# j-dong/rust-raytrace

Measured on AMD Instinct MI355X. Metric: Mrays/sec at 4096x4096, 1000 spheres, depth 8; fraction of HBM roofline, higher is better.
Workload: dtype f64

## Files before the change

include/raytrace_amd.h:

```cpp
#ifndef RAYTRACE_AMD_H
#define RAYTRACE_AMD_H

#include <stddef.h>
#include <stdint.h>

#ifdef __cplusplus
extern "C" {
#endif

#define RT_ABI_VERSION 8

enum rt_status {
    RT_OK = 0,
    RT_E_INVALID = -1,
    RT_E_NODEVICE = -2,
    RT_E_HIP = -3,
    RT_E_NOMEM = -4,
    RT_E_UNSUPPORTED = -5,
    RT_E_PARSE = -6,
    RT_E_NOSCENE = -7,
    RT_E_IO = -8
};

enum rt_shape_kind { RT_SHAPE_SPHERE = 0, RT_SHAPE_PLANE = 1 };
enum rt_material_kind {
    RT_MAT_PHONG = 0, RT_MAT_INDIRECT_PHONG = 1, RT_MAT_FRESNEL = 2, RT_MAT_TRANSPARENT = 3
};
enum rt_light_kind { RT_LIGHT_POINT = 0, RT_LIGHT_DIRECTIONAL = 1, RT_LIGHT_AREA = 2 };
enum rt_camera_kind { RT_CAMERA_SIMPLE = 0, RT_CAMERA_DOF = 1 };
enum rt_background_kind { RT_BG_SOLID = 0, RT_BG_SKYBOX = 1 };

typedef struct { double r, g, b; } rt_color;

// ... 124 lines not shown
void rt_render_opts_default(rt_render_opts* o, uint32_t width, uint32_t height);

int rt_render(rt_ctx* ctx, const rt_render_opts* opts, float* out_rgb, uint8_t* out_bgr, rt_stats* stats);
int rt_render_device(rt_ctx* ctx, const rt_render_opts* opts, void* d_rgb, void* d_bgr, void* stream);
int rt_ctx_reserve(rt_ctx* ctx, const rt_render_opts* opts, int host, void* stream);
int rt_ctx_stats(rt_ctx* ctx, rt_stats* stats);
typedef struct rt_accum rt_accum;

int rt_accum_create(rt_ctx* ctx, const rt_render_opts* opts, rt_accum** out);
void rt_accum_destroy(rt_accum* acc);
int rt_accum_samples(const rt_accum* acc, uint32_t* samples);
int rt_accum_reset(rt_accum* acc);
int rt_render_accumulate(rt_ctx* ctx, rt_accum* acc, uint32_t n_samples, int32_t algo, uint32_t flags, void* stream);
int rt_accum_resolve(rt_ctx* ctx, rt_accum* acc, uint32_t bgr_pitch, void* d_rgb, void* d_bgr, void* stream);
int rt_accum_resolve_host(rt_ctx* ctx, rt_accum* acc, uint32_t bgr_pitch, float* out_rgb, uint8_t* out_bgr);
int rt_accum_download(rt_ctx* ctx, rt_accum* acc, double* sums, size_t cap_doubles, uint32_t* samples);
int rt_accum_upload(rt_ctx* ctx, rt_accum* acc, const double* sums, size_t n_doubles, uint32_t samples);
int rt_checkpoint_write(const char* path, const rt_render_opts* opts, uint64_t scene_hash, uint32_t samples, const double* sums, size_t n_doubles);
int rt_checkpoint_read(const char* path, rt_render_opts* opts, uint64_t* scene_hash, uint32_t* samples, double* sums, size_t cap_doubles);
int rt_div_a2_check(rt_ctx* ctx, const double* x, const double* a, uint32_t n, double* fast, double* slow);
int rt_sqrt_check(rt_ctx* ctx, const double* x, uint32_t n, double* fast, double* slow);
int rt_cull_check(rt_ctx* ctx, uint32_t n, const double* rays, const float* boxes, const double* t, const int32_t* codes,
                  double reach, int32_t* out_i, float* out_f);
double rt_cull_reach(double extent);
int rt_ctx_generation_counts(rt_ctx* ctx, uint32_t* queue, uint32_t* shaded, int n);
enum rt_kernel_family {
    RT_KF_NEAREST = 0,
    RT_KF_OCCLUSION = 1,
    RT_KF_SHADE = 2,
    RT_KF_FOLD = 3,
    RT_KF_TALLY = 4,
    RT_KF_CAMERA = 5,
    RT_KF_COMPOSE = 6,
    RT_KF_TAIL = 7,
    RT_KF_COUNT = 8
};
int rt_ctx_kernel_times(rt_ctx* ctx, double* ms, uint32_t* launches, int n);

int rt_ctx_set_tuning(rt_ctx* ctx, const char* key, int64_t value);
int rt_ctx_get_tuning(const rt_ctx* ctx, const char* key, int64_t* value);
const char* rt_tuning_key(int index);

#ifdef __cplusplus
}
#endif
#endif
// ... 1 lines not shown
```

rust-raytrace_amd/csrc/launch_api.hpp:

```cpp
#pragma once
#include <hip/hip_runtime.h>

#include <cstdint>
#include <vector>

#include "device_layout.hpp"

namespace rtamd {

enum KernelFamily : int8_t {
    kKfNearest = 0, kKfOcclusion = 1, kKfShade = 2, kKfFold = 3, kKfTally = 4, kKfCamera = 5, kKfCompose = 6, kKfTail = 7, kKfCount = 8
};

struct LaunchInterval {
    int start, end;
    KernelFamily fam;
};

struct LaunchMarks {
    std::vector<hipEvent_t>* pool = nullptr;
    int* used = nullptr;
    std::vector<LaunchInterval>* out = nullptr;
    int prev = -1;
    static constexpr int kMaxEvents = 1 << 16;
// ... 44 lines not shown
    hipEvent_t sp_cam = nullptr, sp_ready = nullptr;
    uint32_t *sp_bits = nullptr, *sp_cnt = nullptr, *sp_off = nullptr;
    uint8_t* sp_bgr = nullptr;
    float* sp_rgb = nullptr;
};
hipError_t launch_wavefront(const DevScene& sc, const FrameParams& fp, const WfBufs& b, int src, int src_occ,
                            bool count, const WfStreams& ws, hipEvent_t mark, int mark_gen);
hipError_t upload_srgb_table(const double* avg255);
hipError_t launch_tally(const FrameParams& fp, const WfBufs& b, int n_lights, int generations, hipStream_t s);
constexpr int kDjFlags = 4, kDjWords = 8;
hipError_t launch_signal(uint64_t* flag, uint64_t n, hipStream_t s);
hipError_t launch_join(uint64_t* flags, uint32_t mask, uint64_t n, uint64_t* err, hipStream_t s);
constexpr uint32_t kSegPx = 16;
hipError_t launch_chain_segs(const FrameParams& fp, const WfBufs& b, uint32_t* segbits, uint32_t* rowcnt, uint32_t* rowoff,
                             hipStream_t s);
hipError_t launch_chain_pack(const FrameParams& fp, const uint32_t* segbits, const uint32_t* rowoff, uint8_t* pk_bgr,
                             float* pk_rgb, hipStream_t s);
hipError_t launch_warmup(uint32_t workgroups, hipStream_t s);
hipError_t launch_path_warmup(hipStream_t s);
hipError_t launch_div_a2_probe(const double* x, const double* a, uint32_t n, double* fast, double* slow, hipStream_t s);
hipError_t launch_sqrt_probe(const double* x, uint32_t n, double* fast, double* slow, hipStream_t s);
hipError_t launch_cull_probe(uint32_t n, const double* rays, const float* boxes, const double* t, const int32_t* codes,
                             float reach, int32_t* out_i, float* out_f, hipStream_t s);

size_t path_lds_bytes(const DevScene& sc, bool staged);
int path_waves_per_simd();
hipError_t launch_path(const DevScene& sc, const FrameParams& fp, const PathStack& st, bool staged, hipStream_t stream,
                       bool accumulate = false);
hipError_t launch_accum_resolve(const FrameParams& fp, uint32_t workgroups, hipStream_t s);

}
```

rust-raytrace_amd/csrc/probes.hip:

```cpp
#include <hip/hip_runtime.h>

#include <algorithm>
#include <cstdint>

#include "device_layout.hpp"
#include "launch_api.hpp"
#include "trace_common.hpp"
#include "wf_launch.hpp"

namespace rtamd {

__global__ __launch_bounds__(256) void div_a2_probe(const double* x, const double* a, uint32_t n, double* fast,
                                                    double* slow) {
    for (uint32_t i = blockIdx.x * 256u + threadIdx.x; i < n; i += gridDim.x * 256u) {
        const SphK k = sphere_k(a[i]);
        fast[i] = div_a2(x[i], k);
        slow[i] = x[i] / (2.0 * a[i]);
    }
}

__global__ __launch_bounds__(256) void sqrt_probe(const double* x, uint32_t n, double* fast, double* slow) {
    for (uint32_t i = blockIdx.x * 256u + threadIdx.x; i < n; i += gridDim.x * 256u) {
        fast[i] = sqrt_win(x[i]);
        slow[i] = sqrt(x[i]);
    }
}

__global__ __launch_bounds__(256) void cull_probe(uint32_t n, const double* rays, const float* boxes, const double* t,
                                                  const int32_t* codes, float reach, int32_t* out_i, float* out_f) {
    for (uint32_t i = blockIdx.x * 256u + threadIdx.x; i < n; i += gridDim.x * 256u) {
        const double* q = rays + 6ull * i;
        Ray r;
        r.ox = q[0]; r.oy = q[1]; r.oz = q[2]; r.dx = q[3]; r.dy = q[4]; r.dz = q[5];
        const float* B = boxes + 6ull * i;
        const float lo[3] = {B[0], B[1], B[2]}, hi[3] = {B[3], B[4], B[5]};
        const RayBox rb = make_raybox(r, reach);
        const float tl = t_limit(rb, t[i]);
        float tn, tn_nf;
        const bool hit = box_hit(lo, hi, rb, tl, tn);
        const bool lx = near_is_lo(rb.ix), ly = near_is_lo(rb.iy), lz = near_is_lo(rb.iz);
        const bool hit_nf = box_hit_nf(lx ? lo[0] : hi[0], ly ? lo[1] : hi[1], lz ? lo[2] : hi[2], lx ? hi[0] : lo[0],
                                       ly ? hi[1] : lo[1], lz ? hi[2] : lo[2], rb, tl, tn_nf);
        const uint32_t e16 = stk_entry_c<16>(codes[i], tn), e18 = stk_entry_c<18>(codes[i], tn);
        int32_t* oi = out_i + 5ull * i;
        float* of = out_f + 5ull * i;
        oi[0] = rb.te; oi[1] = hit ? 1 : 0; oi[2] = hit_nf ? 1 : 0; oi[3] = stk_node_c<16>(e16); oi[4] = stk_node_c<18>(e18);
        of[0] = tl; of[1] = tn; of[2] = tn_nf; of[3] = stk_t_c<16>(e16); of[4] = stk_t_c<18>(e18);
    }
}

hipError_t launch_cull_probe(uint32_t n, const double* rays, const float* boxes, const double* t, const int32_t* codes,
                             float reach, int32_t* out_i, float* out_f, hipStream_t s) {
    const uint32_t blocks = std::max(1u, std::min(4096u, (n + 255u) / 256u));
    hipLaunchKernelGGL(cull_probe, dim3(blocks), dim3(256), 0, s, n, rays, boxes, t, codes, reach, out_i, out_f);
    return hipGetLastError();
}

hipError_t launch_sqrt_probe(const double* x, uint32_t n, double* fast, double* slow, hipStream_t s) {
    const uint32_t blocks = std::max(1u, std::min(4096u, (n + 255u) / 256u));
    hipLaunchKernelGGL(sqrt_probe, dim3(blocks), dim3(256), 0, s, x, n, fast, slow);
    return hipGetLastError();
}

hipError_t launch_div_a2_probe(const double* x, const double* a, uint32_t n, double* fast, double* slow, hipStream_t s) {
    const uint32_t blocks = std::max(1u, std::min(4096u, (n + 255u) / 256u));
    hipLaunchKernelGGL(div_a2_probe, dim3(blocks), dim3(256), 0, s, x, a, n, fast, slow);
    return hipGetLastError();
}

RT_UNIT_WARM(probes)

}
```

rust-raytrace_amd/csrc/rt_device.cpp:

```cpp
#include <cstring>
#include <new>
#include <string>

#include "rt_ctx.hpp"

using namespace rtamd;

extern "C" {

int rt_device_count(int* n) {
    if (!n) return RT_E_INVALID;
    *n = 0;
    int k = 0;
    hipError_t e = hipGetDeviceCount(&k);
    if (e != hipSuccess) { *n = 0; return RT_OK; }
    *n = k;
    return RT_OK;
}

int rt_ctx_create(int device, rt_ctx** out) {
    if (!out) return RT_E_INVALID;
    *out = nullptr;
    int n = 0;
    if (hipGetDeviceCount(&n) != hipSuccess || device < 0 || device >= n)
// ... 95 lines not shown
        const size_t o_t = 48 * N, o_box = o_t + 8 * N, o_code = o_box + 24 * N, o_oi = o_code + 4 * N, o_of = o_oi + 20 * N;
        uint8_t* d = nullptr;
        HIP_TRY(c, hipMalloc(&d, o_of + 20 * N));
        auto body = [&]() -> int {
            HIP_TRY(c, hipMemcpyAsync(d, rays, 48 * N, hipMemcpyHostToDevice, c->stream));
            HIP_TRY(c, hipMemcpyAsync(d + o_t, t, 8 * N, hipMemcpyHostToDevice, c->stream));
            HIP_TRY(c, hipMemcpyAsync(d + o_box, boxes, 24 * N, hipMemcpyHostToDevice, c->stream));
            HIP_TRY(c, hipMemcpyAsync(d + o_code, codes, 4 * N, hipMemcpyHostToDevice, c->stream));
            HIP_TRY(c, launch_cull_probe(n, reinterpret_cast<const double*>(d), reinterpret_cast<const float*>(d + o_box),
                                         reinterpret_cast<const double*>(d + o_t), reinterpret_cast<const int32_t*>(d + o_code),
                                         static_cast<float>(reach), reinterpret_cast<int32_t*>(d + o_oi), reinterpret_cast<float*>(d + o_of),
                                         c->stream));
            HIP_TRY(c, hipMemcpyAsync(out_i, d + o_oi, 20 * N, hipMemcpyDeviceToHost, c->stream));
            HIP_TRY(c, hipMemcpyAsync(out_f, d + o_of, 20 * N, hipMemcpyDeviceToHost, c->stream));
            HIP_TRY(c, hipStreamSynchronize(c->stream));
            return RT_OK;
        };
        const int rc = body();
        (void)hipFree(d);
        return rc;
    });
}

int rt_sqrt_check(rt_ctx* c, const double* x, uint32_t n, double* fast, double* slow) {
    if (!c || (n && (!x || !fast || !slow))) return RT_E_INVALID;
    if (n == 0) return RT_OK;
    return guarded(c, [&] {
        HIP_TRY(c, hipSetDevice(c->device));
        const size_t bytes = static_cast<size_t>(n) * sizeof(double);
        double* d = nullptr;
        HIP_TRY(c, hipMalloc(&d, 3 * bytes));
        auto body = [&]() -> int {
            HIP_TRY(c, hipMemcpyAsync(d, x, bytes, hipMemcpyHostToDevice, c->stream));
            HIP_TRY(c, launch_sqrt_probe(d, n, d + n, d + 2 * static_cast<size_t>(n), c->stream));
            HIP_TRY(c, hipMemcpyAsync(fast, d + n, bytes, hipMemcpyDeviceToHost, c->stream));
            HIP_TRY(c, hipMemcpyAsync(slow, d + 2 * static_cast<size_t>(n), bytes, hipMemcpyDeviceToHost, c->stream));
            HIP_TRY(c, hipStreamSynchronize(c->stream));
            return RT_OK;
        };
        const int rc = body();
        (void)hipFree(d);
        return rc;
    });
}

int rt_ctx_set_tuning(rt_ctx* c, const char* key, int64_t value) {
// ... 27 lines not shown
```

rust-raytrace_amd/csrc/trace_common.hpp:

```cpp
#pragma once

#include <hip/hip_runtime.h>

#include <cstdint>
#include <type_traits>

#include "device_layout.hpp"

namespace rtamd {

#ifdef RT_UNIT
#define RT_CAT_(a, b) a##b
#define RT_CAT(a, b) RT_CAT_(a, b)
#define c_srgb_avg RT_CAT(c_srgb_avg_, RT_UNIT)
__constant__ double c_srgb_avg[255];
#else
extern __constant__ double c_srgb_avg[255];
#endif

constexpr double kMinSignificance = 1.0 / 256.0 / 2.0;
constexpr double kEps = 0.00001;
constexpr double kFrac1Pi = 0.318309886183790671537767526745028724;

struct Ray {
// ... 1062 lines not shown
    const double px = ((static_cast<double>(x) + jx) - fp.hw) * fp.scale;
    const double py = ((static_cast<double>(y) + jy) - fp.hh) * fp.scale;
    const double* M = sc.cam_m;
    const double dx = M[0] * px + M[1] * py + M[2] * 1.0;
    const double dy = M[3] * px + M[4] * py + M[5] * 1.0;
    const double dz = M[6] * px + M[7] * py + M[8] * 1.0;
#if RT_DIVK
    const DivK l = div_k(sqrt_win(dx * dx + dy * dy + dz * dz));
    return Ray{sc.cam_pos[0], sc.cam_pos[1], sc.cam_pos[2], div_by(dx, l), div_by(dy, l), div_by(dz, l)};
#else
    const double l = sqrt(dx * dx + dy * dy + dz * dz);
    return Ray{sc.cam_pos[0], sc.cam_pos[1], sc.cam_pos[2], dx / l, dy / l, dz / l};
#endif
}

__device__ __forceinline__ Ray reflect_ray(const Ray& r, double ptx, double pty, double ptz, double nx, double ny,
                                           double nz) {
    const double dn = r.dx * nx + r.dy * ny + r.dz * nz;
    const double k2 = 2.0 * dn;
    const double rdx = r.dx - nx * k2, rdy = r.dy - ny * k2, rdz = r.dz - nz * k2;
    return Ray{ptx + rdx * kEps, pty + rdy * kEps, ptz + rdz * kEps, rdx, rdy, rdz};
}

__device__ __forceinline__ Col average_samples(Col c, uint32_t spp) {
    c = Col{(0.0 + c.r) / 1.0, (0.0 + c.g) / 1.0, (0.0 + c.b) / 1.0};
    Col res{0.0, 0.0, 0.0};
    for (uint32_t k = 0; k < spp; ++k) res = Col{res.r + c.r, res.g + c.g, res.b + c.b};
    const double aa = static_cast<double>(spp);
    return Col{res.r / aa, res.g / aa, res.b / aa};
}

__device__ __forceinline__ void write_pixel(const FrameParams& fp, uint32_t lx, uint32_t out_row, Col res,
                                            const double* srgb = c_srgb_avg) {
    const size_t p = static_cast<size_t>(out_row) * fp.tile_w + lx;
    if (fp.out_rgb) {
        fp.out_rgb[3 * p + 0] = static_cast<float>(res.r);
        fp.out_rgb[3 * p + 1] = static_cast<float>(res.g);
        fp.out_rgb[3 * p + 2] = static_cast<float>(res.b);
    }
    if (fp.out_bgr) {
        uint8_t* q = fp.out_bgr + static_cast<size_t>(out_row) * fp.bgr_pitch + 3u * lx;
        q[0] = to_srgb(res.b, srgb);
        q[1] = to_srgb(res.g, srgb);
        q[2] = to_srgb(res.r, srgb);
        if (lx == fp.tile_w - 1)
            for (uint32_t k = 3u * fp.tile_w; k < fp.pad_end; ++k)
                fp.out_bgr[static_cast<size_t>(out_row) * fp.bgr_pitch + k] = 0;
    }
// ... 60 lines not shown
```

rust-raytrace_amd/csrc/wf_device.hpp:

```cpp
#pragma once
#include <hip/hip_runtime.h>

#include <cstdint>

#include "device_layout.hpp"
#include "trace_common.hpp"

namespace rtamd {
namespace {


__device__ __forceinline__ uint32_t lds_append(uint32_t* counter, bool want) {
    const unsigned long long mask = __ballot(want);
    if (mask == 0) return 0xFFFFFFFFu;
    const int lane = threadIdx.x & 63;
    const int leader = __ffsll(static_cast<long long>(mask)) - 1;
    uint32_t base = 0;
    if (lane == leader) base = atomicAdd(counter, static_cast<uint32_t>(__popcll(mask)));
    base = __shfl(base, leader, 64);
    const uint32_t below = static_cast<uint32_t>(__popcll(mask & ((1ull << lane) - 1ull)));
    return want ? base + below : 0xFFFFFFFFu;
}

__device__ __forceinline__ bool deal_major(const WfBufs& b, uint32_t n) { return b.wg_major && n >= b.spread_below; }
// ... 33 lines not shown
    __syncthreads();
    if (t == 0) {
        uint32_t acc = 0;
        for (int w = 0; w < kT / 64; ++w) { const uint32_t x = s_wave[w]; s_wave[w] = acc; acc += x; }
    }
    __syncthreads();
    uint32_t run = s_wave[wave] + inc - sum;
    for (uint32_t e = 0; e < per; ++e) {
        const uint32_t i = t * per + e;
        if (i < G) s_scan[i] = run;
        run += v[e];
    }
    if (t == kT - 1) s_scan[G] = run;
    __syncthreads();
}

__device__ __forceinline__ size_t region_entry(const uint32_t* s_scan, uint32_t G, uint32_t R, uint32_t i) {
    uint32_t lo = 0, hi = G - 1;
    while (lo < hi) {
        const uint32_t mid = (lo + hi + 1) >> 1;
        if (s_scan[mid] <= i) lo = mid; else hi = mid - 1;
    }
    return static_cast<size_t>(lo) * R + (i - s_scan[lo]);
}

__device__ __forceinline__ bool slot_pixel(const WfBufs& b, const FrameParams& fp, uint32_t j, uint32_t& lx, uint32_t& ly) {
    const uint32_t tile = j >> 6, w = j & 63u;
    lx = (tile % b.tiles_x) * 8u + (w & 7u);
    ly = (tile / b.tiles_x) * 8u + (w >> 3);
    return lx < fp.tile_w && ly < fp.rows;
}

#ifndef RT_NT
#define RT_NT 1
#endif
template <class T>
__device__ __forceinline__ T ldn(const T* p) {
#if RT_NT
    return __builtin_nontemporal_load(p);
#else
    return *p;
#endif
}
template <class T, class U>
__device__ __forceinline__ void stn(T* p, U v) {
#if RT_NT
// ... 356 lines not shown
```

rust-raytrace_amd/csrc/wf_fold.hip:

```cpp
#define RT_UNIT wf_fold
#include <hip/hip_runtime.h>

#include <cstdint>

#include "wf_chain.hpp"
#include "wf_launch.hpp"

namespace rtamd {

namespace {

template <bool kFresnel, bool kAa = false, bool kPack = false>
__global__ __launch_bounds__(RT_FOLD_THREADS, RT_FOLD_WAVES) void wf_fold(DevScene sc, FrameParams fp, WfBufs b, uint32_t lo,
                                                                          uint32_t hi) {
    constexpr int kT = RT_FOLD_THREADS;
    __shared__ double s_srgb[255];
    __shared__ uint32_t s_scan[kMaxRegions + 1];
    __shared__ uint32_t s_wave[kT / 64];
    for (int i = threadIdx.x; i < 255; i += kT) s_srgb[i] = c_srgb_avg[i];
    region_scan<kT>(b.rs(), b.G, s_scan, s_wave);
    const uint32_t n = s_scan[b.G];
    const uint32_t W = gridDim.x * (kT / 64), lane = threadIdx.x & 63u;
    struct Head {
        uint32_t c, nlev, p;
        Col term;
    };
    auto head = [&](uint64_t j) {
        Head hd{0u, kNlevRunning, 0u, Col{0.0, 0.0, 0.0}};
        if (j < n) {
            hd.c = static_cast<uint32_t>(region_entry(s_scan, b.G, b.R, static_cast<uint32_t>(j)));
            hd.nlev = b.nlev()[hd.c];
            hd.p = b.compose ? 0u : b.cpix()[hd.c];
            hd.term = Col{ldn_if<kNtFold>(&b.term(0)[hd.c]), ldn_if<kNtFold>(&b.term(1)[hd.c]),
                          ldn_if<kNtFold>(&b.term(2)[hd.c])};
        }
        return hd;
    };
    uint32_t rc = blockIdx.x * (kT / 64) + (threadIdx.x >> 6);
    Head cur = head(static_cast<uint64_t>(rc) * 64u + lane);
    for (; static_cast<uint64_t>(rc) * 64u < n; rc += W) {
        const Head nxt = head(static_cast<uint64_t>(rc + W) * 64u + lane);
        if (cur.nlev >= lo && cur.nlev <= hi) {
            const Col folded = fold_levels<kFresnel, kPack>(sc, b, cur.c, static_cast<int>(cur.nlev), cur.term);
            const Col res = kAa ? aa_sample(folded) : average_samples(folded, fp.spp);
            emit_chain<kAa>(fp, b, cur.c, cur.p, res, s_srgb);
        }
        cur = nxt;
    }
}

__global__ __launch_bounds__(RT_FOLD_THREADS) void wf_sky_term(DevScene sc, WfBufs b) {
    constexpr int kT = RT_FOLD_THREADS;
    __shared__ uint32_t s_scan[kMaxRegions + 1];
    __shared__ uint32_t s_wave[kT / 64];
    region_scan<kT>(b.rs(), b.G, s_scan, s_wave);
    const uint32_t n = s_scan[b.G];
    for (uint64_t j = static_cast<uint64_t>(blockIdx.x) * kT + threadIdx.x; j < n; j += static_cast<uint64_t>(gridDim.x) * kT) {
        const uint32_t c = static_cast<uint32_t>(region_entry(s_scan, b.G, b.R, static_cast<uint32_t>(j)));
        const uint32_t nl = b.nlev()[c];
        if (nl == kNlevRunning || !(nl & kNlevSky)) continue;
        const Col col = background(sc, Ray{0.0, 0.0, 0.0, b.term(0)[c], b.term(1)[c], b.term(2)[c]});
        b.term(0)[c] = col.r; b.term(1)[c] = col.g; b.term(2)[c] = col.b;
        b.nlev()[c] = static_cast<uint8_t>(nl & ~kNlevSky);
    }
}

}

hipError_t launch_fold(const DevScene& sc, const FrameParams& fp, const WfBufs& b, hipStream_t s, LaunchMarks* m,
                       uint32_t lo, uint32_t hi, bool packed) {
    hipError_t e;
    const dim3 grid(b.G * (kWfThreads / RT_FOLD_THREADS)), block(RT_FOLD_THREADS);
    if (sc.skybox) {
        if (m && (e = m->begin(s)) != hipSuccess) return e;
        hipLaunchKernelGGL(wf_sky_term, grid, block, 0, s, sc, b);
        if (m && (e = m->mark(s, kKfCompose)) != hipSuccess) return e;
    }
    if (m && (e = m->begin(s)) != hipSuccess) return e;
    (void)dispatch_bools(
        [&](auto kFresnel, auto kAa, auto kPack) {
            hipLaunchKernelGGL((wf_fold<kFresnel(), kAa(), kPack()>), grid, block, 0, s, sc, fp, b, lo, hi);
// ... 11 lines not shown
```

rust-raytrace_amd/csrc/wf_nearest.hpp:

```cpp
#pragma once
#include "wf_device.hpp"
#include "wf_launch.hpp"

namespace rtamd {

#ifndef RT_STAMP
#define RT_STAMP 0
#endif
#if RT_STAMP
static __device__ unsigned long long g_stamp[kMaxGenerations][12];
static __device__ unsigned long long g_stamp2[kMaxGenerations][4];
#define RT_STAMP_AT(v)                                                            \
    do {                                                                          \
        asm volatile("s_waitcnt vmcnt(0) lgkmcnt(0)" ::: "memory");              \
        v = __builtin_amdgcn_s_memtime();                                         \
    } while (0)
#define RT_UNIT_STAMPS(unit)                                                                                          \
    hipError_t unit_stamps_##unit(unsigned long long (*a)[12], unsigned long long (*b)[4], bool reset) {              \
        hipError_t e;                                                                                                 \
        if ((e = hipMemcpyFromSymbol(a, HIP_SYMBOL(g_stamp), sizeof g_stamp)) != hipSuccess) return e;                \
        if ((e = hipMemcpyFromSymbol(b, HIP_SYMBOL(g_stamp2), sizeof g_stamp2)) != hipSuccess) return e;              \
        if (!reset) return hipSuccess;                                                                                \
        static unsigned long long za[kMaxGenerations][12], zb[kMaxGenerations][4];                                    \
        if ((e = hipMemcpyToSymbol(HIP_SYMBOL(g_stamp), za, sizeof za)) != hipSuccess) return e;                      \
// ... 39 lines not shown
                double nx, ny, nz;
                hit_normal(sc, sph, h.prim, ptx, pty, ptz, nx, ny, nz);
                const double nd = nx * r.dx + ny * r.dy + nz * r.dz;
                const Shading sh = shading_flags<kFresnel>(m, sig, nd);
                if (!sh.diffuse && !sh.specular) {
                    ends = true;
                    end_obj = h.obj;
                } else {
                    shade = true;
                    if (sh.specular) {
                        if (nd > 0.0) { nx = -nx; ny = -ny; nz = -nz; }
                        rr = reflect_ray(r, ptx, pty, ptz, nx, ny, nz);
                        nsig = (sh.f * sig) * m.ks_sig;
                        refl = true;
                    }
                }
            }
        }
    }
    if (ends) {
        if constexpr (kCam) {
            if (b.compose) stn(&b.pmap()[p], kPixAmbient | static_cast<uint32_t>(end_obj));
            else if constexpr (kAa) aa_add(fp, p, aa_sample(end_colour(sc, end_obj)));
            else write_pixel(fp, p % fp.tile_w, fp.row0 + p / fp.tile_w, average_samples(end_colour(sc, end_obj), fp.spp));
        } else {
            set_terminal(b, p, end_colour(sc, end_obj), k);
        }
    }
    if constexpr (kCam) {
        if (b.mark && live) stn(&b.cmark()[p], static_cast<uint8_t>(shade ? 1 : 0));
        if constexpr (kSky) {
            if (!b.compose && live) stn(&b.csky()[p], static_cast<uint8_t>(h.obj == INT32_MAX ? 1 : 0));
        }
    }
    const uint32_t slot = lds_append(&counts[0], shade);
    const uint32_t chain = kCam ? static_cast<uint32_t>(obase) + slot : p;
    if (kCam && shade && b.compose) stn(&b.pmap()[p], chain);
    if (shade) {
        const size_t at = rbase + slot;
        stn(&b.rf(0)[at], ptx); stn(&b.rf(1)[at], pty); stn(&b.rf(2)[at], ptz);
        stn(&b.rf(3)[at], r.dx); stn(&b.rf(4)[at], r.dy); stn(&b.rf(5)[at], r.dz);
        stn(&b.rf(6)[at], sig);
        stn(&b.ru(0)[at], static_cast<uint32_t>(h.obj));
        stn(&b.ru(1)[at], static_cast<uint32_t>(h.prim));
        stn(&b.ru(2)[at], chain);
        stn(&b.ru(3)[at], 0u);
        if constexpr (kCam) {
// ... 134 lines not shown
```

rust-raytrace_amd/csrc/wf_shade.hip:

```cpp
#include <hip/hip_runtime.h>

#include <cstdint>

#include "wf_chain.hpp"
#include "wf_launch.hpp"

namespace rtamd {

namespace {

template <int kSrc, bool kCount>
__global__ __launch_bounds__(kWfThreads, Src<kSrc>::waves) void wf_occlusion(DevScene sc, FrameParams fp, WfBufs b, int k) {
    extern __shared__ __attribute__((aligned(16))) unsigned char lds[];
    const QueueLds ql = queue_lds(lds + staged_bytes<kSrc>(sc), b.G);
    region_scan(b.rs() + k * b.G, b.G, ql.scan, ql.wave);
    const uint32_t L = static_cast<uint32_t>(sc.n_lights);
    const uint32_t nrec = ql.scan[b.G], n = nrec * L;
    if (!wg_has_work(b, n)) return;
    const BvhView v = stage_lds<kSrc>(sc, lds);
    __syncthreads();
    Work w;
    const size_t rk = static_cast<size_t>(k) * b.qcap;
    const uint32_t W = b.G * (kWfThreads / 64), lane = threadIdx.x & 63u;
    auto item_at = [&](uint32_t qi, uint32_t& l) {
        l = qi / nrec;
        return rk + region_entry(ql.scan, b.G, b.R, qi - l * nrec);
    };
    uint32_t rc = wave_slot(b, n), lc = 0;
    size_t atc = 0;
    double pc[3] = {0.0, 0.0, 0.0};
    int32_t hc = -1;
    if (static_cast<uint64_t>(rc) * 64u + lane < n) {
        atc = item_at(rc * 64u + lane, lc);
        pc[0] = ldn_if<3>(&b.rf(0)[atc]); pc[1] = ldn_if<3>(&b.rf(1)[atc]); pc[2] = ldn_if<3>(&b.rf(2)[atc]);
        hc = static_cast<int32_t>(b.ru(1)[atc]);
    }
    for (; static_cast<uint64_t>(rc) * 64u < n; rc += W) {
        const uint64_t qn = static_cast<uint64_t>(rc + W) * 64u + lane;
        uint32_t ln = 0;
        size_t atn = 0;
        double pn[3] = {0.0, 0.0, 0.0};
        int32_t hn = -1;
        if (qn < n) {
            atn = item_at(static_cast<uint32_t>(qn), ln);
            pn[0] = ldn_if<3>(&b.rf(0)[atn]); pn[1] = ldn_if<3>(&b.rf(1)[atn]); pn[2] = ldn_if<3>(&b.rf(2)[atn]);
            hn = static_cast<int32_t>(b.ru(1)[atn]);
        }
        const uint32_t qi = rc * 64u + lane;
        const uint32_t l = lc;
        const size_t at = atc;
        const double ptx = pc[0], pty = pc[1], ptz = pc[2];
        const int32_t hint = hc;
        lc = ln; atc = atn; pc[0] = pn[0]; pc[1] = pn[1]; pc[2] = pn[2]; hc = hn;
        if (qi >= n) continue;
        double lx, ly, lz, r2;
        const bool has_range = light_dir(sc.lights[l], ptx, pty, ptz, lx, ly, lz, r2);
        const Ray sray{ptx + lx * kEps, pty + ly * kEps, ptz + lz * kEps, lx, ly, lz};
        bool occluded;
        if constexpr (Src<kSrc>::grid)
            occluded = occluded_lgrid<kCount>(sc, v, sc.lgrid[l], sray, r2, ptx, pty, ptz, hint, &w);
        else
            occluded = has_range && sc.lgrid && sc.lgrid[l].R > 0
                           ? occluded_lgrid<kCount>(sc, v, sc.lgrid[l], sray, r2, ptx, pty, ptz, hint, &w)
                           : occluded_any<kSrc, kCount>(sc, v, sray, has_range, r2, hint, &w);
        if (occluded) atomicOr(&b.ru(3)[at], 1u << l);
    }
    flush_work<kCount>(b, 4, w);
}

template <bool kFresnel, bool kPack = false>
__global__ __launch_bounds__(kWfThreads, RT_SHADE_WAVES) void wf_shade(DevScene sc, FrameParams fp, WfBufs b, int k) {
    __shared__ uint32_t s_scan[kMaxRegions + 1];
    __shared__ uint32_t s_wave[kWfThreads / 64];
    region_scan(b.rs() + k * b.G, b.G, s_scan, s_wave);
    const uint32_t n = s_scan[b.G];
    const size_t rk = static_cast<size_t>(k) * b.qcap;
    const uint32_t W = gridDim.x * (kWfThreads / 64), lane = threadIdx.x & 63u;
    const bool lit = sc.n_lights > 0;
    uint32_t rc = wave_slot(b, n);
    ShadeIn cur{};
    bool have = false;
    if (static_cast<uint64_t>(rc) * 64u + lane < n) {
        cur = shade_load(b, rk + region_entry(s_scan, b.G, b.R, rc * 64u + lane), lit);
        have = true;
    }
    for (; static_cast<uint64_t>(rc) * 64u < n; rc += W) {
        const uint64_t jn = static_cast<uint64_t>(rc + W) * 64u + lane;
        ShadeIn nxt{};
        const bool have_n = jn < n;
        if (have_n) nxt = shade_load(b, rk + region_entry(s_scan, b.G, b.R, static_cast<uint32_t>(jn)), lit);
        if (have) shade_compute<kFresnel, true, kPack>(sc, b, k, cur);
        cur = nxt;
        have = have_n;
    }
}

template <int kSrc>
hipError_t launch_occlusion_src(const DevScene& sc, const FrameParams& fp, const WfBufs& b, int k, bool count, hipStream_t s) {
    const size_t lds = staged_bytes<kSrc>(sc) + queue_lds_bytes(b.G);
    return dispatch_bools(
        [&](auto kCount) {
            hipLaunchKernelGGL((wf_occlusion<kSrc, kCount()>), dim3(b.G), dim3(kWfThreads), lds, s, sc, fp, b, k);
            return hipSuccess;
        },
        count);
}

}

hipError_t launch_shading(const DevScene& sc, const FrameParams& fp, const WfBufs& b, int k, int src_occ, int grid_occ,
                          bool count, bool packed, hipStream_t sb, LaunchMarks* mb) {
    hipError_t e;
    if (sc.n_lights > 0) {
// ... 28 lines not shown
```

rust-raytrace_amd/libraytrace/__init__.py:

```python
import ctypes as C
import os

import numpy as np

_HERE = os.path.dirname(os.path.abspath(__file__))
PKG_DIR = os.path.dirname(_HERE)
LIB_PATH = os.environ.get("RT_LIBRTAMD") or os.path.join(PKG_DIR, "librtamd.so")
HEADER_PATH = os.path.join(os.path.dirname(PKG_DIR), "include", "raytrace_amd.h")

RT_ABI_VERSION = 8
RT_OK = 0
RT_E_INVALID, RT_E_NODEVICE, RT_E_HIP, RT_E_NOMEM = -1, -2, -3, -4
RT_E_UNSUPPORTED, RT_E_PARSE, RT_E_NOSCENE, RT_E_IO = -5, -6, -7, -8
RT_SHAPE_SPHERE, RT_SHAPE_PLANE = 0, 1
RT_MAT_PHONG, RT_MAT_INDIRECT_PHONG, RT_MAT_FRESNEL, RT_MAT_TRANSPARENT = 0, 1, 2, 3
RT_LIGHT_POINT, RT_LIGHT_DIRECTIONAL, RT_LIGHT_AREA = 0, 1, 2
RT_CAMERA_SIMPLE, RT_CAMERA_DOF = 0, 1
RT_BG_SOLID, RT_BG_SKYBOX = 0, 1
RT_OUT_RGB_F32, RT_OUT_BGR_U8, RT_COUNT_WORK, RT_TIME_KERNELS, RT_OUT_FRAME_ROWS = 1, 2, 4, 8, 16
KERNEL_FAMILIES = ("nearest", "occlusion", "shade", "fold", "tally", "camera", "compose", "tail")
RT_ALGO_AUTO, RT_ALGO_BRUTE_LDS, RT_ALGO_BRUTE_GLOBAL, RT_ALGO_WAVEFRONT, RT_ALGO_WAVEFRONT_BRUTE = 0, 1, 2, 3, 4
RT_ALGO_PATH = 5
RT_ALGO_WAVEFRONT_AA = 6
RT_JITTER_CENTER, RT_JITTER_RANDOM = 0, 1
RT_MAX_DEPTH_LIMIT = 30


class RtError(RuntimeError):
    def __init__(self, code, msg):
        super().__init__(f"rt error {code}: {msg}")
        self.code = code


# ... 79 lines not shown
        "rt_render_accumulate": (C.c_int, [C.c_void_p, C.c_void_p, C.c_uint32, C.c_int32, C.c_uint32, C.c_void_p]),
        "rt_accum_resolve": (C.c_int, [C.c_void_p, C.c_void_p, C.c_uint32, C.c_void_p, C.c_void_p, C.c_void_p]),
        "rt_accum_resolve_host": (C.c_int, [C.c_void_p, C.c_void_p, C.c_uint32, P(C.c_float), P(C.c_uint8)]),
        "rt_accum_download": (C.c_int, [C.c_void_p, C.c_void_p, P(C.c_double), C.c_size_t, P(C.c_uint32)]),
        "rt_accum_upload": (C.c_int, [C.c_void_p, C.c_void_p, P(C.c_double), C.c_size_t, C.c_uint32]),
        "rt_checkpoint_write": (C.c_int, [C.c_char_p, P(rt_render_opts), C.c_uint64, C.c_uint32, P(C.c_double),
                                          C.c_size_t]),
        "rt_checkpoint_read": (C.c_int, [C.c_char_p, P(rt_render_opts), P(C.c_uint64), P(C.c_uint32), P(C.c_double),
                                         C.c_size_t]),
        "rt_ctx_generation_counts": (C.c_int, [C.c_void_p, P(C.c_uint32), P(C.c_uint32), C.c_int]),
        "rt_ctx_kernel_times": (C.c_int, [C.c_void_p, P(C.c_double), P(C.c_uint32), C.c_int]),
        "rt_light_grid_candidates": (C.c_int, [C.c_void_p, C.c_int, C.c_int, P(C.c_double), C.c_uint32,
                                               P(C.c_int32), P(C.c_int32), C.c_size_t, P(C.c_int64)]),
        "rt_view_grid_candidates": (C.c_int, [C.c_void_p, C.c_int, P(C.c_double), C.c_uint32, P(C.c_int32),
                                              P(C.c_int32), P(C.c_float), C.c_size_t, P(C.c_int64)]),
        "rt_qtree_nodes": (C.c_int, [C.c_void_p, C.c_int, C.c_void_p, P(C.c_float), P(C.c_int32), P(C.c_int32),
                                     C.c_size_t, P(C.c_int64)]),
        "rt_div_a2_check": (C.c_int, [C.c_void_p, P(C.c_double), P(C.c_double), C.c_uint32, P(C.c_double),
                                      P(C.c_double)]),
        "rt_sqrt_check": (C.c_int, [C.c_void_p, P(C.c_double), C.c_uint32, P(C.c_double), P(C.c_double)]),
        "rt_cull_check": (C.c_int, [C.c_void_p, C.c_uint32, P(C.c_double), P(C.c_float), P(C.c_double), P(C.c_int32),
                                    C.c_double, P(C.c_int32), P(C.c_float)]),
        "rt_cull_reach": (C.c_double, [C.c_double]),
        "rt_ctx_set_tuning": (C.c_int, [C.c_void_p, C.c_char_p, C.c_int64]),
        "rt_ctx_get_tuning": (C.c_int, [C.c_void_p, C.c_char_p, P(C.c_int64)]),
        "rt_tuning_key": (C.c_char_p, [C.c_int]),
    }
    for name, (res, args) in sig.items():
        f = getattr(lib, name)
        f.restype = res
        f.argtypes = args
    if lib.rt_abi_version() != RT_ABI_VERSION:
        raise ImportError(f"{LIB_PATH} has ABI {lib.rt_abi_version()}, these bindings expect {RT_ABI_VERSION}: rebuild")
    return lib


lib = _load()


def _err(ctx=None):
    m = lib.rt_last_error(ctx)
    return m.decode(errors="replace") if m else ""


def _check(rc, ctx=None):
    if rc != RT_OK:
# ... 282 lines not shown
        fast = np.empty_like(x)
        slow = np.empty_like(x)
        P = C.POINTER(C.c_double)
        _check(lib.rt_sqrt_check(self._h, x.ctypes.data_as(P), x.size, fast.ctypes.data_as(P), slow.ctypes.data_as(P)),
               self._h)
        return fast, slow

    def cull_check(self, rays, boxes, t, codes, reach=float("inf")):
        rays = np.ascontiguousarray(rays, dtype=np.float64)
        boxes = np.ascontiguousarray(boxes, dtype=np.float32)
        t = np.ascontiguousarray(t, dtype=np.float64)
        codes = np.ascontiguousarray(codes, dtype=np.int32)
        n = t.size
        assert rays.shape == (n, 6) and boxes.shape == (n, 6) and t.shape == (n,) and codes.shape == (n,)
        oi = np.empty((n, 5), np.int32)
        of = np.empty((n, 5), np.float32)
        PD, PF, PI = C.POINTER(C.c_double), C.POINTER(C.c_float), C.POINTER(C.c_int32)
        _check(lib.rt_cull_check(self._h, n, rays.ctypes.data_as(PD), boxes.ctypes.data_as(PF), t.ctypes.data_as(PD),
                                 codes.ctypes.data_as(PI), float(reach), oi.ctypes.data_as(PI), of.ctypes.data_as(PF)),
               self._h)
        return {"te": oi[:, 0], "hit": oi[:, 1] != 0, "hit_nf": oi[:, 2] != 0, "node16": oi[:, 3], "node18": oi[:, 4],
                "tlim": of[:, 0], "tnear": of[:, 1], "tnear_nf": of[:, 2], "t16": of[:, 3], "t18": of[:, 4]}

    def accumulator(self, opts):
        return Accumulator(self, opts)

    def kernel_times(self):
        n = len(KERNEL_FAMILIES)
        ms = (C.c_double * n)()
        cnt = (C.c_uint32 * n)()
        _check(lib.rt_ctx_kernel_times(self._h, ms, cnt, n), self._h)
        return {f: (ms[i], cnt[i]) for i, f in enumerate(KERNEL_FAMILIES)}

    def close(self):
        if self._h:
            lib.rt_ctx_destroy(self._h)
            self._h = C.c_void_p()

    def __enter__(self):
        return self

    def __exit__(self, *a):
        self.close()

    def __del__(self):
        try:
# ... 101 lines not shown
```

Baseline: 17220.

## Resolve region entries once per wave via ballot search instead of per-lane binary search

Adds a wave-cooperative region lookup: each wave finds the region of its first item with a ballot/popcount over the LDS prefix scan, and when all 64 items fall in one region it computes every lane's entry by offset, skipping the per-lane binary search. The fold, sky, occlusion and shade kernels now use this lookup, and occlusion also narrows its indices to 32 bits and computes the light index uniformly per wave. A single-sample shortcut is added to average_samples, and a probe plus host API for checking lookup correctness is included. In exchange it adds readfirstlane and ballot logic and a fallback path for waves that span region boundaries.

```diff
diff --git a/include/raytrace_amd.h b/include/raytrace_amd.h
--- a/include/raytrace_amd.h
+++ b/include/raytrace_amd.h
@@ -8,7 +8,7 @@
 extern "C" {
 #endif
 
-#define RT_ABI_VERSION 8
+#define RT_ABI_VERSION 9
 
 enum rt_status {
     RT_OK = 0,
@@ -179,6 +179,7 @@
 int rt_sqrt_check(rt_ctx* ctx, const double* x, uint32_t n, double* fast, double* slow);
 int rt_cull_check(rt_ctx* ctx, uint32_t n, const double* rays, const float* boxes, const double* t, const int32_t* codes,
                   double reach, int32_t* out_i, float* out_f);
+int rt_region_lookup_check(rt_ctx* ctx, uint32_t G, uint32_t R, const uint32_t* sizes, uint64_t n, uint64_t* entries);
 double rt_cull_reach(double extent);
 int rt_ctx_generation_counts(rt_ctx* ctx, uint32_t* queue, uint32_t* shaded, int n);
 enum rt_kernel_family {
diff --git a/rust-raytrace_amd/csrc/launch_api.hpp b/rust-raytrace_amd/csrc/launch_api.hpp
--- a/rust-raytrace_amd/csrc/launch_api.hpp
+++ b/rust-raytrace_amd/csrc/launch_api.hpp
@@ -90,6 +90,7 @@
 hipError_t launch_sqrt_probe(const double* x, uint32_t n, double* fast, double* slow, hipStream_t s);
 hipError_t launch_cull_probe(uint32_t n, const double* rays, const float* boxes, const double* t, const int32_t* codes,
                              float reach, int32_t* out_i, float* out_f, hipStream_t s);
+hipError_t launch_region_lookup_probe(const uint32_t* sizes, uint32_t G, uint32_t R, uint64_t n, uint64_t* out, hipStream_t s);
 
 size_t path_lds_bytes(const DevScene& sc, bool staged);
 int path_waves_per_simd();
diff --git a/rust-raytrace_amd/csrc/probes.hip b/rust-raytrace_amd/csrc/probes.hip
--- a/rust-raytrace_amd/csrc/probes.hip
+++ b/rust-raytrace_amd/csrc/probes.hip
@@ -6,6 +6,7 @@
 #include "device_layout.hpp"
 #include "launch_api.hpp"
 #include "trace_common.hpp"
+#include "wf_device.hpp"
 #include "wf_launch.hpp"
 
 namespace rtamd {
@@ -49,6 +50,25 @@
     }
 }
 
+__global__ __launch_bounds__(kWfThreads) void region_lookup_probe(const uint32_t* sizes, uint32_t G, uint32_t R, uint64_t* out) {
+    __shared__ uint32_t s_scan[kMaxScan + 1];
+    __shared__ uint32_t s_wave[kWfThreads / 64];
+    region_scan(sizes, G, s_scan, s_wave);
+    const uint32_t n = s_scan[G], lane = threadIdx.x & 63u;
+    const uint32_t W = gridDim.x * (kWfThreads / 64);
+    for (uint32_t c = blockIdx.x * (kWfThreads / 64) + (threadIdx.x >> 6); static_cast<uint64_t>(c) * 64u < n; c += W) {
+        const uint32_t i0 = c * 64u, cnt = min(64u, n - i0);
+        const size_t at = wave_region_entry(s_scan, G, R, i0, cnt);
+        if (lane < cnt) out[i0 + lane] = at;
+    }
+}
+
+hipError_t launch_region_lookup_probe(const uint32_t* sizes, uint32_t G, uint32_t R, uint64_t n, uint64_t* out, hipStream_t s) {
+    const uint32_t blocks = static_cast<uint32_t>(std::max<uint64_t>(1, std::min<uint64_t>(64, (n + kWfThreads - 1) / kWfThreads)));
+    hipLaunchKernelGGL(region_lookup_probe, dim3(blocks), dim3(kWfThreads), 0, s, sizes, G, R, out);
+    return hipGetLastError();
+}
+
 hipError_t launch_cull_probe(uint32_t n, const double* rays, const float* boxes, const double* t, const int32_t* codes,
                              float reach, int32_t* out_i, float* out_f, hipStream_t s) {
     const uint32_t blocks = std::max(1u, std::min(4096u, (n + 255u) / 256u));
diff --git a/rust-raytrace_amd/csrc/rt_device.cpp b/rust-raytrace_amd/csrc/rt_device.cpp
--- a/rust-raytrace_amd/csrc/rt_device.cpp
+++ b/rust-raytrace_amd/csrc/rt_device.cpp
@@ -141,6 +141,31 @@
     });
 }
 
+int rt_region_lookup_check(rt_ctx* c, uint32_t G, uint32_t R, const uint32_t* sizes, uint64_t n, uint64_t* entries) {
+    if (!c || !sizes || G == 0 || G > static_cast<uint32_t>(kMaxScan) || (n && !entries)) return RT_E_INVALID;
+    uint64_t sum = 0;
+    for (uint32_t r = 0; r < G; ++r) sum += sizes[r];
+    if (sum != n || n > 0xFFFFFFFFull) return fail(c, RT_E_INVALID, "rt_region_lookup_check: n is not the sum of the sizes (below 2^32)");
+    if (n == 0) return RT_OK;
+    return guarded(c, [&] {
+        HIP_TRY(c, hipSetDevice(c->device));
+        const size_t o_out = align_up(static_cast<size_t>(G) * 4, 8);
+        uint8_t* d = nullptr;
+        HIP_TRY(c, hipMalloc(&d, o_out + 8 * static_cast<size_t>(n)));
+        auto body = [&]() -> int {
+            HIP_TRY(c, hipMemcpyAsync(d, sizes, static_cast<size_t>(G) * 4, hipMemcpyHostToDevice, c->stream));
+            HIP_TRY(c, launch_region_lookup_probe(reinterpret_cast<const uint32_t*>(d), G, R, n, reinterpret_cast<uint64_t*>(d + o_out),
+                                                  c->stream));
+            HIP_TRY(c, hipMemcpyAsync(entries, d + o_out, 8 * static_cast<size_t>(n), hipMemcpyDeviceToHost, c->stream));
+            HIP_TRY(c, hipStreamSynchronize(c->stream));
+            return RT_OK;
+        };
+        const int rc = body();
+        (void)hipFree(d);
+        return rc;
+    });
+}
+
 int rt_sqrt_check(rt_ctx* c, const double* x, uint32_t n, double* fast, double* slow) {
     if (!c || (n && (!x || !fast || !slow))) return RT_E_INVALID;
     if (n == 0) return RT_OK;
diff --git a/rust-raytrace_amd/csrc/trace_common.hpp b/rust-raytrace_amd/csrc/trace_common.hpp
--- a/rust-raytrace_amd/csrc/trace_common.hpp
+++ b/rust-raytrace_amd/csrc/trace_common.hpp
@@ -1108,8 +1108,13 @@
     return Ray{ptx + rdx * kEps, pty + rdy * kEps, ptz + rdz * kEps, rdx, rdy, rdz};
 }
 
+#ifndef RT_SPP1
+#define RT_SPP1 1
+#endif
+template <bool kOne = true>
 __device__ __forceinline__ Col average_samples(Col c, uint32_t spp) {
     c = Col{(0.0 + c.r) / 1.0, (0.0 + c.g) / 1.0, (0.0 + c.b) / 1.0};
+    if (kOne && RT_SPP1 && spp == 1) return Col{0.0 + c.r, 0.0 + c.g, 0.0 + c.b};
     Col res{0.0, 0.0, 0.0};
     for (uint32_t k = 0; k < spp; ++k) res = Col{res.r + c.r, res.g + c.g, res.b + c.b};
     const double aa = static_cast<double>(spp);
diff --git a/rust-raytrace_amd/csrc/wf_device.hpp b/rust-raytrace_amd/csrc/wf_device.hpp
--- a/rust-raytrace_amd/csrc/wf_device.hpp
+++ b/rust-raytrace_amd/csrc/wf_device.hpp
@@ -79,6 +79,43 @@
         if (s_scan[mid] <= i) lo = mid; else hi = mid - 1;
     }
     return static_cast<size_t>(lo) * R + (i - s_scan[lo]);
+}
+
+#ifndef RT_WAVE_LOOKUP
+#define RT_WAVE_LOOKUP 1
+#endif
+__device__ __forceinline__ uint32_t wave_region_of(const uint32_t* s_scan, uint32_t G, uint32_t x) {
+    const uint32_t lane = threadIdx.x & 63u;
+    const uint32_t S = (G + 63u) >> 6;
+    const uint32_t ic = lane * S;
+    const bool bc = ic < G && s_scan[ic] <= x;
+    const uint32_t base = (static_cast<uint32_t>(__popcll(__ballot(bc))) - 1u) * S;
+    if (S == 1) return base;
+    const uint32_t jf = base + lane;
+    const bool bf = lane < S && jf < G && s_scan[jf] <= x;
+    return base + static_cast<uint32_t>(__popcll(__ballot(bf))) - 1u;
+}
+
+__device__ __forceinline__ size_t wave_region_entry(const uint32_t* s_scan, uint32_t G, uint32_t R, uint32_t i0, uint32_t cnt) {
+    const uint32_t lane = threadIdx.x & 63u;
+#if RT_WAVE_LOOKUP
+    i0 = __builtin_amdgcn_readfirstlane(i0);
+    cnt = __builtin_amdgcn_readfirstlane(cnt);
+    const uint32_t r0 = wave_region_of(s_scan, G, i0);
+    const uint32_t a0 = __builtin_amdgcn_readfirstlane(s_scan[r0]);
+    const uint32_t e0 = __builtin_amdgcn_readfirstlane(s_scan[r0 + 1]);
+    if (e0 - i0 >= cnt)
+        return static_cast<size_t>(r0) * R + (i0 - a0 + lane);
+    const uint32_t i = i0 + lane;
+    uint32_t lo = r0, hi = wave_region_of(s_scan, G, i0 + cnt - 1u);
+    while (lo < hi) {
+        const uint32_t mid = (lo + hi + 1) >> 1;
+        if (s_scan[mid] <= i) lo = mid; else hi = mid - 1;
+    }
+    return static_cast<size_t>(lo) * R + (i - s_scan[lo]);
+#else
+    return lane < cnt ? region_entry(s_scan, G, R, i0 + lane) : 0;
+#endif
 }
 
 __device__ __forceinline__ bool slot_pixel(const WfBufs& b, const FrameParams& fp, uint32_t j, uint32_t& lx, uint32_t& ly) {
diff --git a/rust-raytrace_amd/csrc/wf_fold.hip b/rust-raytrace_amd/csrc/wf_fold.hip
--- a/rust-raytrace_amd/csrc/wf_fold.hip
+++ b/rust-raytrace_amd/csrc/wf_fold.hip
@@ -25,10 +25,11 @@
         uint32_t c, nlev, p;
         Col term;
     };
-    auto head = [&](uint64_t j) {
+    auto head = [&](uint64_t j0) {
         Head hd{0u, kNlevRunning, 0u, Col{0.0, 0.0, 0.0}};
+        const uint64_t j = j0 + lane;
+        if (j0 < n) hd.c = static_cast<uint32_t>(wave_region_entry(s_scan, b.G, b.R, static_cast<uint32_t>(j0), min(64u, n - static_cast<uint32_t>(j0))));
         if (j < n) {
-            hd.c = static_cast<uint32_t>(region_entry(s_scan, b.G, b.R, static_cast<uint32_t>(j)));
             hd.nlev = b.nlev()[hd.c];
             hd.p = b.compose ? 0u : b.cpix()[hd.c];
             hd.term = Col{ldn_if<kNtFold>(&b.term(0)[hd.c]), ldn_if<kNtFold>(&b.term(1)[hd.c]),
@@ -37,9 +38,9 @@
         return hd;
     };
     uint32_t rc = blockIdx.x * (kT / 64) + (threadIdx.x >> 6);
-    Head cur = head(static_cast<uint64_t>(rc) * 64u + lane);
+    Head cur = head(static_cast<uint64_t>(rc) * 64u);
     for (; static_cast<uint64_t>(rc) * 64u < n; rc += W) {
-        const Head nxt = head(static_cast<uint64_t>(rc + W) * 64u + lane);
+        const Head nxt = head(static_cast<uint64_t>(rc + W) * 64u);
         if (cur.nlev >= lo && cur.nlev <= hi) {
             const Col folded = fold_levels<kFresnel, kPack>(sc, b, cur.c, static_cast<int>(cur.nlev), cur.term);
             const Col res = kAa ? aa_sample(folded) : average_samples(folded, fp.spp);
@@ -55,8 +56,9 @@
     __shared__ uint32_t s_wave[kT / 64];
     region_scan<kT>(b.rs(), b.G, s_scan, s_wave);
     const uint32_t n = s_scan[b.G];
-    for (uint64_t j = static_cast<uint64_t>(blockIdx.x) * kT + threadIdx.x; j < n; j += static_cast<uint64_t>(gridDim.x) * kT) {
-        const uint32_t c = static_cast<uint32_t>(region_entry(s_scan, b.G, b.R, static_cast<uint32_t>(j)));
+    for (uint64_t j0 = static_cast<uint64_t>(blockIdx.x) * kT + (threadIdx.x & ~63u); j0 < n; j0 += static_cast<uint64_t>(gridDim.x) * kT) {
+        const uint32_t c = static_cast<uint32_t>(wave_region_entry(s_scan, b.G, b.R, static_cast<uint32_t>(j0), min(64u, n - static_cast<uint32_t>(j0))));
+        if (j0 + (threadIdx.x & 63u) >= n) continue;
         const uint32_t nl = b.nlev()[c];
         if (nl == kNlevRunning || !(nl & kNlevSky)) continue;
         const Col col = background(sc, Ray{0.0, 0.0, 0.0, b.term(0)[c], b.term(1)[c], b.term(2)[c]});
diff --git a/rust-raytrace_amd/csrc/wf_nearest.hpp b/rust-raytrace_amd/csrc/wf_nearest.hpp
--- a/rust-raytrace_amd/csrc/wf_nearest.hpp
+++ b/rust-raytrace_amd/csrc/wf_nearest.hpp
@@ -85,7 +85,7 @@
         if constexpr (kCam) {
             if (b.compose) stn(&b.pmap()[p], kPixAmbient | static_cast<uint32_t>(end_obj));
             else if constexpr (kAa) aa_add(fp, p, aa_sample(end_colour(sc, end_obj)));
-            else write_pixel(fp, p % fp.tile_w, fp.row0 + p / fp.tile_w, average_samples(end_colour(sc, end_obj), fp.spp));
+            else write_pixel(fp, p % fp.tile_w, fp.row0 + p / fp.tile_w, average_samples<false>(end_colour(sc, end_obj), fp.spp));
         } else {
             set_terminal(b, p, end_colour(sc, end_obj), k);
         }
diff --git a/rust-raytrace_amd/csrc/wf_shade.hip b/rust-raytrace_amd/csrc/wf_shade.hip
--- a/rust-raytrace_amd/csrc/wf_shade.hip
+++ b/rust-raytrace_amd/csrc/wf_shade.hip
@@ -22,33 +22,55 @@
     Work w;
     const size_t rk = static_cast<size_t>(k) * b.qcap;
     const uint32_t W = b.G * (kWfThreads / 64), lane = threadIdx.x & 63u;
-    auto item_at = [&](uint32_t qi, uint32_t& l) {
+    constexpr bool kWave = RT_WAVE_LOOKUP && kSrc != kSrcGridG && kSrc != kSrcBvhL8;
+    auto item_at = [&](uint32_t q0, [[maybe_unused]] uint32_t cnt, uint32_t& l) {
+        if constexpr (kWave) {
+            q0 = __builtin_amdgcn_readfirstlane(q0);
+            cnt = __builtin_amdgcn_readfirstlane(cnt);
+            uint32_t l0 = 0;
+            if (L <= 32u) {
+                for (uint32_t t = 1, m = nrec; t < L; ++t, m += nrec) l0 += q0 >= m ? 1u : 0u;
+            } else {
+                l0 = q0 / nrec;
+            }
+            const uint32_t rec0 = q0 - l0 * nrec;
+            if (cnt <= nrec - rec0) {
+                l = l0;
+                return static_cast<uint32_t>(wave_region_entry(ql.scan, b.G, b.R, rec0, cnt));
+            }
+        }
+        const uint32_t qi = q0 + lane;
         l = qi / nrec;
-        return rk + region_entry(ql.scan, b.G, b.R, qi - l * nrec);
+        return static_cast<uint32_t>(region_entry(ql.scan, b.G, b.R, qi - l * nrec));
     };
     uint32_t rc = wave_slot(b, n), lc = 0;
-    size_t atc = 0;
+    uint32_t atc = 0;
     double pc[3] = {0.0, 0.0, 0.0};
     int32_t hc = -1;
+    if constexpr (kWave)
+        if (static_cast<uint64_t>(rc) * 64u < n) atc = item_at(rc * 64u, min(64u, n - rc * 64u), lc);
     if (static_cast<uint64_t>(rc) * 64u + lane < n) {
-        atc = item_at(rc * 64u + lane, lc);
-        pc[0] = ldn_if<3>(&b.rf(0)[atc]); pc[1] = ldn_if<3>(&b.rf(1)[atc]); pc[2] = ldn_if<3>(&b.rf(2)[atc]);
-        hc = static_cast<int32_t>(b.ru(1)[atc]);
+        if constexpr (!kWave) atc = item_at(rc * 64u, 0u, lc);
+        pc[0] = ldn_if<3>(&b.rf(0)[rk + atc]); pc[1] = ldn_if<3>(&b.rf(1)[rk + atc]); pc[2] = ldn_if<3>(&b.rf(2)[rk + atc]);
+        hc = static_cast<int32_t>(b.ru(1)[rk + atc]);
     }
     for (; static_cast<uint64_t>(rc) * 64u < n; rc += W) {
         const uint64_t qn = static_cast<uint64_t>(rc + W) * 64u + lane;
         uint32_t ln = 0;
-        size_t atn = 0;
+        uint32_t atn = 0;
         double pn[3] = {0.0, 0.0, 0.0};
         int32_t hn = -1;
+        const uint64_t qn0 = static_cast<uint64_t>(rc + W) * 64u;
+        if constexpr (kWave)
+            if (qn0 < n) atn = item_at(static_cast<uint32_t>(qn0), min(64u, n - static_cast<uint32_t>(qn0)), ln);
         if (qn < n) {
-            atn = item_at(static_cast<uint32_t>(qn), ln);
-            pn[0] = ldn_if<3>(&b.rf(0)[atn]); pn[1] = ldn_if<3>(&b.rf(1)[atn]); pn[2] = ldn_if<3>(&b.rf(2)[atn]);
-            hn = static_cast<int32_t>(b.ru(1)[atn]);
+            if constexpr (!kWave) atn = item_at(static_cast<uint32_t>(qn0), 0u, ln);
+            pn[0] = ldn_if<3>(&b.rf(0)[rk + atn]); pn[1] = ldn_if<3>(&b.rf(1)[rk + atn]); pn[2] = ldn_if<3>(&b.rf(2)[rk + atn]);
+            hn = static_cast<int32_t>(b.ru(1)[rk + atn]);
         }
         const uint32_t qi = rc * 64u + lane;
         const uint32_t l = lc;
-        const size_t at = atc;
+        const uint32_t at = atc;
         const double ptx = pc[0], pty = pc[1], ptz = pc[2];
         const int32_t hint = hc;
         lc = ln; atc = atn; pc[0] = pn[0]; pc[1] = pn[1]; pc[2] = pn[2]; hc = hn;
@@ -63,7 +85,7 @@
             occluded = has_range && sc.lgrid && sc.lgrid[l].R > 0
                            ? occluded_lgrid<kCount>(sc, v, sc.lgrid[l], sray, r2, ptx, pty, ptz, hint, &w)
                            : occluded_any<kSrc, kCount>(sc, v, sray, has_range, r2, hint, &w);
-        if (occluded) atomicOr(&b.ru(3)[at], 1u << l);
+        if (occluded) atomicOr(&b.ru(3)[rk + at], 1u << l);
     }
     flush_work<kCount>(b, 4, w);
 }
@@ -80,15 +102,18 @@
     uint32_t rc = wave_slot(b, n);
     ShadeIn cur{};
     bool have = false;
+    size_t at = 0;
+    if (static_cast<uint64_t>(rc) * 64u < n) at = wave_region_entry(s_scan, b.G, b.R, rc * 64u, min(64u, n - rc * 64u));
     if (static_cast<uint64_t>(rc) * 64u + lane < n) {
-        cur = shade_load(b, rk + region_entry(s_scan, b.G, b.R, rc * 64u + lane), lit);
+        cur = shade_load(b, rk + at, lit);
         have = true;
     }
     for (; static_cast<uint64_t>(rc) * 64u < n; rc += W) {
-        const uint64_t jn = static_cast<uint64_t>(rc + W) * 64u + lane;
+        const uint64_t jn0 = static_cast<uint64_t>(rc + W) * 64u, jn = jn0 + lane;
         ShadeIn nxt{};
         const bool have_n = jn < n;
-        if (have_n) nxt = shade_load(b, rk + region_entry(s_scan, b.G, b.R, static_cast<uint32_t>(jn)), lit);
+        if (jn0 < n) at = wave_region_entry(s_scan, b.G, b.R, static_cast<uint32_t>(jn0), min(64u, n - static_cast<uint32_t>(jn0)));
+        if (have_n) nxt = shade_load(b, rk + at, lit);
         if (have) shade_compute<kFresnel, true, kPack>(sc, b, k, cur);
         cur = nxt;
         have = have_n;
diff --git a/rust-raytrace_amd/libraytrace/__init__.py b/rust-raytrace_amd/libraytrace/__init__.py
--- a/rust-raytrace_amd/libraytrace/__init__.py
+++ b/rust-raytrace_amd/libraytrace/__init__.py
@@ -8,7 +8,7 @@
 LIB_PATH = os.environ.get("RT_LIBRTAMD") or os.path.join(PKG_DIR, "librtamd.so")
 HEADER_PATH = os.path.join(os.path.dirname(PKG_DIR), "include", "raytrace_amd.h")
 
-RT_ABI_VERSION = 8
+RT_ABI_VERSION = 9
 RT_OK = 0
 RT_E_INVALID, RT_E_NODEVICE, RT_E_HIP, RT_E_NOMEM = -1, -2, -3, -4
 RT_E_UNSUPPORTED, RT_E_PARSE, RT_E_NOSCENE, RT_E_IO = -5, -6, -7, -8
@@ -134,6 +134,7 @@
         "rt_cull_check": (C.c_int, [C.c_void_p, C.c_uint32, P(C.c_double), P(C.c_float), P(C.c_double), P(C.c_int32),
                                     C.c_double, P(C.c_int32), P(C.c_float)]),
         "rt_cull_reach": (C.c_double, [C.c_double]),
+        "rt_region_lookup_check": (C.c_int, [C.c_void_p, C.c_uint32, C.c_uint32, P(C.c_uint32), C.c_uint64, P(C.c_uint64)]),
         "rt_ctx_set_tuning": (C.c_int, [C.c_void_p, C.c_char_p, C.c_int64]),
         "rt_ctx_get_tuning": (C.c_int, [C.c_void_p, C.c_char_p, P(C.c_int64)]),
         "rt_tuning_key": (C.c_char_p, [C.c_int]),
@@ -462,6 +463,15 @@
         return {"te": oi[:, 0], "hit": oi[:, 1] != 0, "hit_nf": oi[:, 2] != 0, "node16": oi[:, 3], "node18": oi[:, 4],
                 "tlim": of[:, 0], "tnear": of[:, 1], "tnear_nf": of[:, 2], "t16": of[:, 3], "t18": of[:, 4]}
 
+    def region_lookup_check(self, sizes, R):
+        sizes = np.ascontiguousarray(sizes, dtype=np.uint32)
+        assert sizes.ndim == 1
+        n = int(sizes.sum(dtype=np.uint64))
+        out = np.empty(n, np.uint64)
+        _check(lib.rt_region_lookup_check(self._h, sizes.size, int(R), sizes.ctypes.data_as(C.POINTER(C.c_uint32)), n,
+                                          out.ctypes.data_as(C.POINTER(C.c_uint64))), self._h)
+        return out
+
     def accumulator(self, opts):
         return Accumulator(self, opts)
 
```

After: 17270, median of 6. No clear change (+0.3%).
